# hyunjik11/GPT

Hardware: AMD Instinct MI355X
Metric: SGLD steps/sec (kin40k, n_feat=500/dim, r=5) (higher is better)
Workload: dtype f64

## Files before the change

gpt_amd/csrc/chain.hip:

```cpp
#include "device_util.h"

namespace gpt {

constexpr int kChainBufs = 1;
constexpr int kChainDMax = 8;
constexpr int kChainTPW8 = 1;
constexpr int kChainTasks = 2;
constexpr int kChainG = 2;
constexpr int kChainQPL = 4;
constexpr int kChainQP = 64 * kChainQPL;
constexpr int kChainRun = 64;
constexpr int kChainRunS = 72;
constexpr int kChainQS = 264;

constexpr int kChainMMax = 256;

GPT_HD constexpr int chain_scratch_dbl(int r) {
  const int s0a = 7 * 4 * r * r, s0b = 64 * 8;
  return (s0a > s0b ? s0a : s0b) + 2 * r * r + 3 * r * r + r;
}
GPT_HD constexpr int al16c(int x) { return (x + 15) & ~15; }

template <int R, int G, int WV = kChainDMax>
struct ChainLds {
  static constexpr int DRG = kChainDMax * R * G;
  static constexpr int TS = 2 * (DRG + G);
  static constexpr int NTMAX = kChainQPL * G;
  static constexpr int o_IT = 0;
  static constexpr int o_w = al16c(o_IT + 4 * kChainQP * kChainDMax);
  static constexpr int o_idx = al16c(o_w + 8 * kChainQP);
  static constexpr int o_y = al16c(o_idx + 4 * kChainMMax);
  static constexpr int o_temp = al16c(o_y + 8 * kChainMMax);
  static constexpr int o_fp = al16c(o_temp + 8 * 2 * TS);
  static constexpr int o_gwp = al16c(o_fp + 8 * kChainQPL * G);
  static constexpr int o_misc = al16c(o_gwp + 8 * NTMAX * 64);
  static constexpr int o_touch = al16c(o_misc + 8 * 16);
  static constexpr int o_un = al16c(o_touch + 256);
  static constexpr int L_dbl = G * kChainQS + WV * G * R * kChainRunS;
  static constexpr int x_dbl = chain_scratch_dbl(R);
  static constexpr int o_tab = al16c(o_un + 8 * (L_dbl > x_dbl * WV ? L_dbl : x_dbl * WV));
  static constexpr bool tab = WV == kChainDMax;
  static constexpr int bytes = al16c(o_tab + (tab ? 8 * 64 : 0));
};

#ifndef CHAIN_TIMELINE
#define CHAIN_TIMELINE 2
#endif

#ifndef CHAIN_SSTAMP
#define CHAIN_SSTAMP 0
#endif
#ifndef CHAIN_STAMPS
#define CHAIN_STAMPS CHAIN_SSTAMP
#endif
#define CHAIN_FENCE() do {} while (0)
#ifndef CHAIN_PRIO
#define CHAIN_PRIO 2
#endif
#define CHAIN_SETPRIO(hi_upper)                                                             \
  do {                                                                                      \
    if (CHAIN_PRIO) {                                                                       \
      if ((k >= 4) == (hi_upper)) __builtin_amdgcn_s_setprio(1);                            \
      else __builtin_amdgcn_s_setprio(0);                                                   \
    }                                                                                       \
  } while (0)
#if !CHAIN_STAMPS
#define CSTAMP(slot) CHAIN_FENCE()
#endif
#if CHAIN_TIMELINE
#define TSTAMP_ANY(i)                                                                       \
  do {                                                                                      \
    if (P.tline && tid == 0 && (i) < kTimelineSteps + 2) {                                  \
      long long* ts_ = P.tline + (size_t)blockIdx.x * kTimeline + 2 * (i);                  \
      ts_[0] = (long long)__builtin_amdgcn_s_memrealtime();                                \
      ts_[1] = (long long)__builtin_amdgcn_s_memtime();                                    \
    }                                                                                       \
  } while (0)
#else
#define TSTAMP_ANY(i) do {} while (0)
#endif
#if CHAIN_TIMELINE == 1
#define TSTAMP(i) TSTAMP_ANY(i)
#else
#define TSTAMP(i) do {} while (0)
#endif
#if CHAIN_STAMPS
#define CSTAMP(slot)                                                                        \
  do {                                                                                      \
    if (P.stamps && tid == 0)                                                               \
      P.stamps[(size_t)blockIdx.x * kStamps + (slot)] = (long long)__builtin_amdgcn_s_memtime(); \
  } while (0)
#endif

#if CHAIN_STAMPS
#define LSTAMP(slot)                                                                        \
  do {                                                                                      \
    if (P.stamps && g0 == 20 && lane == 0 && (k == 0 || k == 4))                            \
      P.stamps[(size_t)(gridDim.x + blockIdx.x) * kStamps + (k ? 8 : 0) + (slot)] =         \
          (long long)__builtin_amdgcn_s_memtime();                                         \
  } while (0)
#else
#define LSTAMP(slot) CHAIN_FENCE()
#endif

#define SSTAMP(slot)                                                                        \
  do {                                                                                      \
    if ((slot) == 4) CHAIN_SETPRIO(false);        \
    if ((slot) == 7) CHAIN_SETPRIO(true);        \
    if (CHAIN_SSTAMP && P.stamps && lane == 0 && (k == 0 || k == 4))                                        \
      P.stamps[(size_t)((2 + (slot) / 8) * gridDim.x + blockIdx.x) * kStamps + (k ? 8 : 0) + \
               (slot) % 8] = (long long)__builtin_amdgcn_s_memtime();                       \
  } while (0)

__device__ __forceinline__ void lds_barrier() {
  asm volatile("s_waitcnt lgkmcnt(0)\n\ts_barrier" ::: "memory");
}

template <int R, int J, int G, int WV>
__global__ __launch_bounds__(64 * WV, WV == 4 ? 2 : 1) void chain_kernel(StepParams P,
                                                                const ChainDesc* chains,
                                                                const long long* __restrict__ tbase,
                                                                int t_local, int nsteps) {
  extern __shared__ __attribute__((aligned(16))) unsigned char smem[];
  __shared__ __attribute__((aligned(16))) double pbuf[kChainBufs * WV * G * 64 * J];
  const ChainDesc* Cp = chains + blockIdx.x;
  const int tid = threadIdx.x, lane = tid & 63, k = uni(tid >> 6);
  const int n = P.n, D = P.D, Q = P.Q, m = P.m, NTH = 64 * D;
  using L = ChainLds<R, G, WV>;
  const int NCH = (Q + 63) / 64, NT = NCH * G;
  int* IT_l = (int*)(smem + L::o_IT);
  double* w_l = (double*)(smem + L::o_w);
  int* idx_l = (int*)(smem + L::o_idx);
  double* y_l = (double*)(smem + L::o_y);
  double* temp_l = (double*)(smem + L::o_temp);
  double* fp_l = (double*)(smem + L::o_fp);
  double* gwp_l = (double*)(smem + L::o_gwp);
  double* misc = (double*)(smem + L::o_misc);
  int* flag = (int*)(misc + 8);
  double* wVr = (double*)(smem + L::o_un);
  double* X = (double*)(smem + L::o_un) + k * L::x_dbl;
  double* xi_l = X;
  double* pw0 = pbuf + k * (kChainBufs * G * 64 * J);
  [[maybe_unused]] double* bscr = wVr + G * kChainQS + k * G * R * kChainRunS;

  TSTAMP_ANY(0);
#if CHAIN_TIMELINE
  if (P.tline && tid == 0) {
    long long* ts_ = P.tline + (size_t)blockIdx.x * kTimeline + kTimeline - 2;
    ts_[0] = (long long)__builtin_amdgcn_s_getreg((31 << 11) | 4);
    ts_[1] = (long long)__builtin_amdgcn_s_getreg((31 << 11) | 20);
  }
#endif
  const long long t0 = tbase[0] + t_local;
  if (t0 >= P.total_steps) return;
  if (__hip_atomic_load(Cp->status, __ATOMIC_RELAXED, __HIP_MEMORY_SCOPE_AGENT) != 0) return;
  CSTAMP(0);
  const long long tend = min(P.total_steps, t0 + (long long)nsteps);

  auto batch_of = [&](long long tt, int& bt) -> const int32_t* {
    const int ee = (int)(tt / P.nb), bb = (int)(tt - (long long)ee * P.nb);
    bt = min(m, P.N - bb * m);
    return Cp->order + (size_t)(ee & 1) * P.N + (size_t)bb * m;
  };
  long long t = t0;
  int Bt;
  const int32_t* ord = batch_of(t, Bt);
  const long long koff = (long long)n * k, rstride = (long long)n * D;
  const double* phi_k = uni_ptr(Cp->phi) + koff;
  auto stage_rows = [&](const int (&rows)[G], int ln, double* pw) {
#pragma unroll
    for (int gg = 0; gg < G; ++gg) {
      const char* rb = (const char*)(phi_k + (long long)rows[gg] * rstride);
      __attribute__((address_space(3))) double* dst =
          (__attribute__((address_space(3))) double*)(pw + gg * 64 * J);
      if constexpr (J >= 2) {
#pragma unroll
        for (int s = 0; s < J / 2; ++s) {
          const unsigned o = min(16u * ln + 1024u * s, 8u * n - 16u);
          __builtin_amdgcn_global_load_lds((const __attribute__((address_space(1))) void*)(rb + o),
                                           (__attribute__((address_space(3))) void*)(dst + 128 * s),
                                           16, 0, 0);
        }
      } else {
#pragma unroll
        for (int s = 0; s < 2; ++s) {
          const unsigned o = min(4u * ln + 256u * s, 8u * n - 4u);
          __builtin_amdgcn_global_load_lds((const __attribute__((address_space(1))) void*)(rb + o),
                                           (__attribute__((address_space(3))) void*)(dst + 32 * s),
                                           4, 0, 0);
        }
      }
    }
// ... 149 lines not shown
      const double wV = ok ? wq * V : 0.0;
      if (ok) wVr[gg * kChainQS + q] = wV;
      vsave[x] = ok ? V : 0.0;
      const double fs = wave_sum(wV);
      if (lane == 0) fp_l[gg * kChainQPL + c] = fs;
    }
    LSTAMP(5);
    lds_barrier();
    LSTAMP(6);
    double res[G];
#pragma unroll
    for (int gg = 0; gg < G; ++gg) {
      double f = fp_l[gg * kChainQPL];
#pragma unroll
      for (int c = 1; c < kChainQPL; ++c) f += fp_l[gg * kChainQPL + c];
      res[gg] = (g0 + gg < Bt) ? y_l[g0 + gg] - f : 0.0;
    }
#pragma unroll
    for (int gg = 0; gg < G; ++gg) {
      const double* wr = wVr + gg * kChainQS;
      double a = wr[gq[0] & 0xffff];
#pragma unroll
      for (int i = 1; i < 8; ++i) a += wr[(gq[i >> 1] >> (16 * (i & 1))) & 0xffff];
      a = (group8_sum(a) * tsl[DRG + G + (k * R + rl) * G + gg]) * res[gg];
      double cc[R];
#pragma unroll
      for (int l = 0; l < R; ++l) cc[l] = readlane_d(a, 8 * l);
#pragma unroll
      for (int jj = 0; jj < J; ++jj) {
        const double pv = p[gg][jj];
#pragma unroll
        for (int l = 0; l < R; ++l) acc[jj][l] = fma(pv, cc[l], acc[jj][l]);
      }
    }
#pragma unroll
    for (int x = 0; x < TPW; ++x) {
      const int task = k + D * x;
      if (task >= NT) break;
      const int gg = task / NCH;
      double rr = res[0];
#pragma unroll
      for (int g2 = 1; g2 < G; ++g2) if (gg == g2) rr = res[g2];
      gw[x] = fma(vsave[x], rr, gw[x]);
    }
    LSTAMP(7);
  }
  CSTAMP(2);

  const ChainDesc* Cq = Cp;
  asm volatile("" : "+s"(Cq));
  const ChainDesc C = *Cq;
  const double cN = (double)P.N / (double)Bt;
  const long long post = t - P.burnin_steps;
  const bool store = post >= 0 && ((post + 1) % P.store_every) == 0;
  const long long slot_s = store ? (post + 1) / P.store_every - 1 : 0;

#pragma unroll
  for (int x = 0; x < TPW; ++x) {
    const int task = k + D * x;
    if (task >= NT) break;
    gwp_l[task * 64 + lane] = gw[x];
  }
  SSTAMP(0);
  __syncthreads();
  SSTAMP(1);
  CHAIN_SETPRIO(true);
  {
    const double inv_sw2 = 1.0 / (C.sigma_w * C.sigma_w);
    const double sqe = sqrt(C.epsw);
    double gn2 = 0.0;
#pragma unroll 1
    for (int q = tid; q < Q; q += NTH) {
      const int c = q >> 6, ln = q & 63;
      double g = 0.0;
      for (int gg = 0; gg < G; ++gg) g += gwp_l[(gg * NCH + c) * 64 + ln];
      const double wq = w_l[q];
      const double gradw = cN * g / C.signal_var - wq * inv_sw2;
      double step = C.epsw * gradw / 2;
      step += sqe * normal_at(C.seed, (uint32_t)q, (uint32_t)t, kWNoise, 0);
      const double wn = wq + step;
      w_l[q] = wn;
      if (t + 1 == tend) gptr_w(C.w)[(size_t)((t + 1) & 1) * Q + q] = wn;
      if (store && C.w_store) gptr_w(C.w_store)[(size_t)slot_s * Q + q] = wn;
      gn2 = fma(gradw, gradw, gn2);
    }
    if (C.diag) {
      gn2 = wave_sum(gn2);
      if (lane == 0) misc[k] = gn2;
    }
  }
  SSTAMP(2);
  int Bn = 0;
  const int32_t* ordn = nullptr;
  if (t + 1 < tend) {
    ordn = batch_of(t + 1, Bn);
    for (int i = tid; i < Bn; i += NTH) {
      const int row = gptr(ordn)[i];
      idx_l[i] = row;
      y_l[i] = gptr(Cp->y)[row];
    }
    int rows0[G];
#pragma unroll
    for (int gg = 0; gg < G; ++gg) rows0[gg] = gptr(ordn)[min(gg, Bn - 1)];
    stage_rows(rows0, lane, pw0);
  }
  CSTAMP(3);
  SSTAMP(3);

  const double cU = cN / C.signal_var;
  const double sq = sqrt(C.epsU);
  double gu2 = 0.0;
  {
    constexpr int NQJ = (J + 3) / 4;
    constexpr int NZ = J >= 4 ? 4 : 2;
    const int NQ = unoise_nq(n);
#pragma unroll 1
    for (int l = 0; l < R; ++l) {
#pragma unroll
      for (int q = 0; q < NQJ; ++q) {
        double z[4];
        if constexpr (L::tab)
          normal_quad_tab<NZ>(C.seed, (uint32_t)((l * NQ + q) * 64 + lane), (uint32_t)t, kUNoise,
                              (uint32_t)k, (const double*)(smem + L::o_tab), z);
        else
          normal_quad<NZ>(C.seed, (uint32_t)((l * NQ + q) * 64 + lane), (uint32_t)t, kUNoise,
                          (uint32_t)k, z);
#pragma unroll
        for (int i = 0; i < NZ; ++i)
          if (4 * q + i < J) xi_l[(4 * q + i) * 64 + lane] = z[i];
      }
#pragma unroll
      for (int L = 0; L < R; ++L) {
        if (l == L) {
#pragma unroll
          for (int jj = 0; jj < J; ++jj) {
            const int j = lane + 64 * jj;
            const double Gv = j < n ? acc[jj][L] * cU : 0.0;
            gu2 = fma(Gv, Gv, gu2);
            acc[jj][L] = j < n ? sq * Gv / 2 + xi_l[jj * 64 + lane] : 0.0;
          }
        }
      }
    }
  }
  if (C.diag) {
    gu2 = wave_sum(gu2);
    if (lane == 0) C.diag[(size_t)t * (1 + D) + 1 + k] = sqrt(gu2);
  }
  CSTAMP(4);
  SSTAMP(4);
  {
    constexpr int NN = 2 * R;
    constexpr int S0 = (7 * NN * NN > 64 * 8) ? 7 * NN * NN : 64 * 8;
    double* X0 = X;
    double* Ec = X + S0;
    double* Mg = Ec + NN * R;
    double* Ag = Mg + R * R;
    double* Sg = Ag + R * R;
    double* nr = Sg + R * R;
    wave_sync();
#pragma unroll
    for (int a = 0; a < R; ++a) {
      double v[R];
#pragma unroll
      for (int bb = 0; bb < R; ++bb) {
        double s0 = 0.0;
#pragma unroll
        for (int jj = 0; jj < J; ++jj) s0 = fma(u[jj][a], acc[jj][bb], s0);
        v[bb] = s0;
      }
      wave_sum_to_lds<R>(v, Mg + a * R);
    }
    wave_sync();
    SSTAMP(5);
#pragma unroll
    for (int bb = 0; bb < R; ++bb) {
      double ms[R];
#pragma unroll
      for (int a = 0; a < R; ++a) ms[a] = Mg[a * R + bb] + Mg[bb * R + a];
#pragma unroll
      for (int jj = 0; jj < J; ++jj) {
        double s = 0.0;
#pragma unroll
        for (int a = 0; a < R; ++a) s = fma(u[jj][a], ms[a], s);
        acc[jj][bb] = acc[jj][bb] - s / 2;
      }
    }
      CSTAMP(5);
      SSTAMP(6);
      {
#pragma unroll
        for (int a = 0; a < R; ++a) {
          double v[R];
#pragma unroll
          for (int bb = 0; bb < R; ++bb) {
            double s1 = 0.0;
            if (bb >= a)
#pragma unroll
              for (int jj = 0; jj < J; ++jj) s1 = fma(acc[jj][a], acc[jj][bb], s1);
            v[bb] = s1;
          }
          wave_sum_to_lds<R>(v, Sg + a * R);
        }
        wave_sync();
        for (int o = lane; o < R * R; o += 64) {
          const int i = o / R, b = o - i * R;
          Ag[o] = (Mg[o] - Mg[b * R + i]) / 2;
          if (i > b) Sg[o] = Sg[b * R + i];
        }
      }
      wave_sync();
      const double tt = sq;
      for (int o = lane; o < NN * NN; o += 64) {
        const int i = o / NN, j = o - i * NN;
        double v;
        if (i < R) v = j < R ? Ag[i * R + j] : -Sg[i * R + (j - R)];
        else v = j < R ? (i - R == j ? 1.0 : 0.0) : Ag[(i - R) * R + (j - R)];
        X0[o] = tt * v;
      }
      wave_sync();
      long long* xst = (CHAIN_SSTAMP && P.stamps && k == 0)
                           ? P.stamps + (size_t)(4 * gridDim.x + blockIdx.x) * kStamps : nullptr;
      const bool bad = wave_expm<NN>(X0, xst);
      SSTAMP(7);
      for (int o = lane; o < NN * R; o += 64) {
        const int a = o / R, l = o - a * R;
        Ec[o] = X0[NN * NN + a * NN + l];
      }
      wave_sync();
      double* X1 = X0;
      for (int o = lane; o < R * R; o += 64) X1[o] = -tt * Ag[o];
      wave_sync();
      wave_expm<R>(X1, xst ? xst + (size_t)gridDim.x * kStamps : nullptr);
      if (bad && lane == 0) flag[0] = 1;
      CSTAMP(6);
      SSTAMP(8);
      const double* mx = X1 + R * R;
      double* F = Mg;
      wave_sync();
      for (int o = lane; o < NN * R; o += 64) {
        const int a = o / R, l = o - a * R;
        double s = 0.0;
#pragma unroll
        for (int c2 = 0; c2 < R; ++c2) s = fma(Ec[a * R + c2], mx[c2 * R + l], s);
        F[o] = s;
      }
      wave_sync();
      SSTAMP(9);
      {
        double Fh[R * R];
#pragma unroll
        for (int x = 0; x < R * R; ++x) Fh[x] = F[x];
#pragma unroll
        for (int jj = 0; jj < J; ++jj) {
          double o[R];
#pragma unroll
          for (int l = 0; l < R; ++l) o[l] = 0.0;
#pragma unroll
          for (int a = 0; a < R; ++a)
#pragma unroll
            for (int l = 0; l < R; ++l) o[l] = fma(u[jj][a], Fh[a * R + l], o[l]);
#pragma unroll
          for (int l = 0; l < R; ++l) u[jj][l] = o[l];
        }
      }
      SSTAMP(10);
      double nrm[R];
#pragma unroll
      for (int l = 0; l < R; ++l) nrm[l] = 0.0;
      {
        double Fh[R * R];
#pragma unroll
        for (int x = 0; x < R * R; ++x) Fh[x] = F[R * R + x];
#pragma unroll
        for (int jj = 0; jj < J; ++jj) {
#pragma unroll
          for (int a = 0; a < R; ++a)
#pragma unroll
            for (int l = 0; l < R; ++l) u[jj][l] = fma(acc[jj][a], Fh[a * R + l], u[jj][l]);
#pragma unroll
          for (int l = 0; l < R; ++l) nrm[l] = fma(u[jj][l], u[jj][l], nrm[l]);
        }
      }
      SSTAMP(11);
      wave_sum_to_lds<R>(nrm, nr);
      wave_sync();
      SSTAMP(12);
#pragma unroll
      for (int l = 0; l < R; ++l) {
        const double isc = 1.0 / sqrt(nr[l]);
#pragma unroll
        for (int jj = 0; jj < J; ++jj) u[jj][l] = u[jj][l] * isc;
      }
    }
    SSTAMP(13);
    if (CHAIN_PRIO) __builtin_amdgcn_s_setprio(0);
    if (CHAIN_STAMPS && P.stamps && lane == 0)
    P.stamps[(size_t)blockIdx.x * kStamps + 8 + k] = (long long)__builtin_amdgcn_s_memtime();
  __syncthreads();
    if (C.diag && tid == 0) {
      double s = 0.0;
      for (int w2 = 0; w2 < D; ++w2) s += misc[w2];
      C.diag[(size_t)t * (1 + D)] = sqrt(s);
    }
    if (flag[0]) {
      if (tid == 0) __hip_atomic_store(C.status, 1, __ATOMIC_RELAXED, __HIP_MEMORY_SCOPE_AGENT);
      return;
    }
    double* Uk = (t + 1 == tend) ? C.U + (size_t)n * R * k : nullptr;
    double* Us = (store && C.U_store) ? C.U_store + ((size_t)slot_s * D + k) * n * R : nullptr;
#pragma unroll
    for (int jj = 0; jj < J; ++jj) {
      const int j = lane + 64 * jj;
      if (j < n)
#pragma unroll
        for (int l = 0; l < R; ++l) {
          if (Uk) gptr_w(Uk)[j + (size_t)n * l] = u[jj][l];
          if (Us) gptr_w(Us)[j + (size_t)n * l] = u[jj][l];
        }
    }
    CSTAMP(7);
    SSTAMP(15);
    TSTAMP(2 + (int)(t - t0));
    if (++t >= tend) break;
    ord = ordn;
    Bt = Bn;
  }
#if CHAIN_TIMELINE == 2
  TSTAMP_ANY(2 + (int)(tend - 1 - t0));
#endif
}

static_assert(contains(ChainWVs{}, kChainDMax), "the wide U phase has one wave per dimension");

static int chain_wv(int D) { return D <= 4 ? 4 : kChainDMax; }
static size_t chain_static_lds(int J, int WV) { return 8 * (size_t)kChainBufs * WV * kChainG * 64 * J; }

static int chain_J(int n) { return n <= 64 ? 1 : (n <= 128 ? 2 : (n <= 256 ? 4 : (n <= 512 ? 8 : 0))); }

size_t chain_lds_bytes(int n, int D, int r, int Q, int m) {
  (void)n; (void)Q; (void)m;
  return with_value_or(ChainRanks{}, r, (size_t)1 << 30, [&](auto R) {
    return with_value_or(ChainWVs{}, chain_wv(D), (size_t)1 << 30, [&](auto WV) {
      return (size_t)ChainLds<R, kChainG, WV>::bytes;
    });
  });
}

bool chain_supported(int n, int D, int r, int Q, int m, bool langevin, bool stiefel, int max_run) {
  if (max_run > kChainRun) return false;
  if (!langevin || !stiefel) return false;
  if (D < 1 || D > kChainDMax || r < 1 || r > 5 || chain_J(n) == 0) return false;
  if (chain_J(n) >= 2 && (n & 1)) return false;
  if (Q > kChainQP || m > kChainMMax) return false;
  const int NT = (Q + 63) / 64 * kChainG;
  if (NT > ((chain_J(n) >= 8 && D > 4) ? kChainTPW8 : kChainTasks) * D) return false;
  return chain_lds_bytes(n, D, r, Q, m) + chain_static_lds(chain_J(n), chain_wv(D)) <= 160 * 1024;
}

hipError_t launch_chain(const StepParams& P, const ChainDesc* chains, int nchains,
                        const long long* tbase, int t_local, int nsteps, hipStream_t st) {
  const int J = chain_J(P.n);
  const size_t lds = chain_lds_bytes(P.n, P.D, P.r, P.Q, P.m);
  dim3 grid(nchains), block(64 * P.D);
  return with_value(ChainRanks{}, P.r, [&](auto R) {
    return with_value(ChainJs{}, J, [&](auto JJ) {
      return with_value(ChainWVs{}, chain_wv(P.D), [&](auto WV) {
        return launch_big_lds<chain_kernel<R, JJ, kChainG, WV>>(
            (int)(kMaxLds - chain_static_lds(JJ, WV)), grid, block, lds, st, P, chains, tbase,
            t_local, nsteps);
      });
    });
  });
}

}
```

gpt_amd/csrc/device_util.h:

```cpp
#pragma once
#include "gpt_internal.h"

namespace gpt {

__device__ __forceinline__ int uni(int x) { return __builtin_amdgcn_readfirstlane(x); }
template <class T>
__device__ __forceinline__ T* uni_ptr(T* p) {
  const unsigned long long v = (unsigned long long)p;
  const unsigned lo = __builtin_amdgcn_readfirstlane((unsigned)v);
  const unsigned hi = __builtin_amdgcn_readfirstlane((unsigned)(v >> 32));
  return (T*)(((unsigned long long)hi << 32) | lo);
}

typedef double d4 __attribute__((ext_vector_type(4)));
typedef double d2 __attribute__((ext_vector_type(2)));

__device__ __forceinline__ void tri_pair(long long t, int& a, int& b) {
  int ta = (int)((sqrt(8.0 * (double)t + 1.0) - 1.0) / 2.0);
  while ((long long)ta * (ta + 1) / 2 > t) --ta;
  while ((long long)(ta + 1) * (ta + 2) / 2 <= t) ++ta;
  a = ta;
  b = (int)(t - (long long)ta * (ta + 1) / 2);
}

// ... 516 lines not shown
        for (int x = 0; x < BS; ++x) {
          a[x] = A[min(i0 + x, NN - 1) * NN + t];
          b[x] = B[t * NN + min(j0 + x, NN - 1)];
        }
#pragma unroll
        for (int x = 0; x < BS; ++x)
#pragma unroll
          for (int y = 0; y < BS; ++y) acc[x][y] = fma(a[x], b[y], acc[x][y]);
      }
#pragma unroll
      for (int x = 0; x < BS; ++x)
#pragma unroll
        for (int y = 0; y < BS; ++y)
          if (i0 + x < NN && j0 + y < NN) C[(i0 + x) * NN + j0 + y] = acc[x][y];
    }
    wave_sync();
    return;
  }
  for (int o = lane; o < NN * NN; o += 64) {
    const int i = o / NN, j = o - i * NN;
    double a[NN], b[NN];
#pragma unroll
    for (int t = 0; t < NN; ++t) { a[t] = A[i * NN + t]; b[t] = B[t * NN + j]; }
    double s = 0.0;
#pragma unroll
    for (int t = 0; t < NN; ++t) s = fma(a[t], b[t], s);
    C[o] = s;
  }
  wave_sync();
}

template <int NN>
__device__ __forceinline__ void wave_solve_body(double* M, double* X, long long* st);
template <int NN>
__device__ __noinline__ void wave_solve_ool(double* M, double* X, long long* st) {
  __builtin_assume(__builtin_amdgcn_is_shared((const __attribute__((address_space(0))) void*)M));
  __builtin_assume(__builtin_amdgcn_is_shared((const __attribute__((address_space(0))) void*)X));
  wave_solve_body<NN>(M, X, st);
}
template <int NN>
__device__ __forceinline__ void wave_solve(double* M, double* X, long long* st = nullptr) {
  if constexpr (NN >= 16) wave_solve_ool<NN>(M, X, st);
  else wave_solve_body<NN>(M, X, st);
}
template <int NN>
__device__ __forceinline__ void wave_solve_body(double* M, double* X, long long* st) {
  const int lane = threadIdx.x & 63;
  bool dd = true;
  if (lane < NN) {
    double off = 0.0;
    for (int i = 0; i < NN; ++i)
      if (i != lane) off += fabs(M[i * NN + lane]);
    dd = fabs(M[lane * NN + lane]) > off;
  }
  const bool nopiv = __all(dd);
  for (int c = 0; c < NN; ++c) {
    int bi = c;
    if (!nopiv) {
      const double mine = (lane >= c && lane < NN) ? fabs(M[lane * NN + c]) : -1.0;
      const double best = wave_max(mine);
      const unsigned long long hit = __ballot(mine == best && lane >= c && lane < NN);
      bi = hit ? (int)__ffsll((long long)hit) - 1 : c;
    }
    if (bi != c) {
      for (int col = lane; col < NN; col += 64) {
        double t0 = M[c * NN + col]; M[c * NN + col] = M[bi * NN + col]; M[bi * NN + col] = t0;
        double t1 = X[c * NN + col]; X[c * NN + col] = X[bi * NN + col]; X[bi * NN + col] = t1;
      }
      wave_sync();
    }
    const double rp = 1.0 / M[c * NN + c];
    const int mcols = NN - c - 1, wcols = mcols + NN;
    if (lane < wcols) {
      const int cb = lane + 64;
      const bool two = cb < wcols;
      double* pa = lane < mcols ? M + (c + 1 + lane) : X + (lane - mcols);
      double* pb = two ? (cb < mcols ? M + (c + 1 + cb) : X + (cb - mcols)) : pa;
      const double piva = pa[c * NN], pivb = pb[c * NN];
      for (int r0 = c + 1; r0 < NN; r0 += 8) {
        double fv[8], ca[8], cbv[8];
#pragma unroll
        for (int u = 0; u < 8; ++u) {
          const int rr = min(r0 + u, NN - 1);
          fv[u] = M[rr * NN + c];
          ca[u] = pa[rr * NN];
          cbv[u] = pb[rr * NN];
        }
#pragma unroll
        for (int u = 0; u < 8; ++u) {
          const double f = fv[u] * rp;
          if (r0 + u < NN) {
            pa[(r0 + u) * NN] = ca[u] - f * piva;
            if (two) pb[(r0 + u) * NN] = cbv[u] - f * pivb;
          }
        }
      }
    }
    wave_sync();
  }
  if (st && lane == 0) st[15] = (long long)__builtin_amdgcn_s_memtime();
  for (int col = lane; col < NN; col += 64) {
    double x[NN];
#pragma unroll
    for (int t = 0; t < NN; ++t) x[t] = X[t * NN + col];
#pragma unroll
    for (int c = NN - 1; c >= 0; --c) {
      double s = x[c];
#pragma unroll
      for (int t = c + 1; t < NN; ++t) s -= M[c * NN + t] * x[t];
      x[c] = s / M[c * NN + c];
    }
#pragma unroll
    for (int t = 0; t < NN; ++t) X[t * NN + col] = x[t];
  }
  wave_sync();
}

template <int NV>
__device__ __forceinline__ void wave_sum_to_lds(double (&v)[NV], double* dst) {
  constexpr int NB = NV <= 8 ? 8 : (NV <= 16 ? 16 : (NV <= 32 ? 32 : 64));
  const int lane = lane_id();
  double b[NB];
#pragma unroll
  for (int x = 0; x < NB; ++x) b[x] = x < NV ? v[x] : 0.0;
  Butterfly<NB>::run(b, lane);
  constexpr int SH = 6 - Butterfly<NB>::P;
  const int vi = lane >> SH;
  if ((lane & ((1 << SH) - 1)) == 0 && vi < NV) dst[vi] = b[0];
}
template <int NV>
__device__ __forceinline__ void wave_sum_to_lds(double (&v)[2 * NV], double* dst, double* dst2) {
  constexpr int NB = 2 * NV <= 8 ? 8 : (2 * NV <= 16 ? 16 : (2 * NV <= 32 ? 32 : 64));
  const int lane = lane_id();
  double b[NB];
#pragma unroll
  for (int x = 0; x < NB; ++x) b[x] = x < 2 * NV ? v[x] : 0.0;
  Butterfly<NB>::run(b, lane);
  constexpr int SH = 6 - Butterfly<NB>::P;
  const int vi = lane >> SH;
  if ((lane & ((1 << SH) - 1)) == 0 && vi < 2 * NV) {
    if (vi < NV) dst[vi] = b[0];
    else dst2[vi - NV] = b[0];
  }
}

__device__ __forceinline__ double readlane_d(double v, int lane) {
  const long long b = __double_as_longlong(v);
  const int lo = __builtin_amdgcn_readlane((int)(b & 0xffffffffLL), lane);
  const int hi = __builtin_amdgcn_readlane((int)(b >> 32), lane);
  return __longlong_as_double(((long long)hi << 32) | (unsigned int)lo);
}

template <int NN>
__device__ __forceinline__ bool wave_solve_dd(const double* M, double* X) {
  const int lane = threadIdx.x & 63;
  bool dd = true;
  if (lane < NN) {
    double off = 0.0;
#pragma unroll
    for (int i = 0; i < NN; ++i)
      if (i != lane) off += fabs(M[i * NN + lane]);
    dd = fabs(M[lane * NN + lane]) > off;
  }
  if (!__all(dd)) return false;
  double col[NN];
#pragma unroll
  for (int i = 0; i < NN; ++i) {
    const int c = lane < NN ? lane : lane - NN;
    col[i] = lane < NN ? M[i * NN + c] : (lane < 2 * NN ? X[i * NN + c] : 0.0);
  }
  double rpv[NN];
#pragma unroll
  for (int p = 0; p < NN; ++p) {
    const double rp = rcp_nr(readlane_d(col[p], p));
    rpv[p] = rp;
#pragma unroll
    for (int i = p + 1; i < NN; ++i) {
      const double f = readlane_d(col[i], p) * rp;
      col[i] -= f * col[p];
    }
  }
  const bool xl = lane >= NN;
#pragma unroll
  for (int k = NN - 1; k >= 0; --k) {
    double u[NN];
#pragma unroll
    for (int i = 0; i < k; ++i) u[i] = readlane_d(col[i], k);
    if (xl) {
      col[k] = col[k] * rpv[k];
#pragma unroll
      for (int i = 0; i < k; ++i) col[i] -= col[k] * u[i];
    }
  }
  wave_sync();
  if (lane >= NN && lane < 2 * NN) {
#pragma unroll
    for (int i = 0; i < NN; ++i) X[i * NN + lane - NN] = col[i];
  }
  wave_sync();
  return true;
}

template <int NN>
__device__ __noinline__ bool wave_solve_dd2(const double* Mg, double* Xg, double* Fg) {
  static_assert(NN > 32 && NN <= 64, "two-pass register LU");
  typedef __attribute__((address_space(3))) double lds_d;
  const lds_d* M = (const lds_d*)Mg;
  lds_d* X = (lds_d*)Xg;
  lds_d* F = (lds_d*)Fg;
  const int lane = lane_id();
  bool dd = true;
  if (lane < NN) {
    double off = 0.0;
#pragma unroll
    for (int i = 0; i < NN; ++i)
      if (i != lane) off += fabs(M[i * NN + lane]);
    dd = fabs(M[lane * NN + lane]) > off;
  }
  if (!__all(dd)) return false;
  double col[NN];
#pragma unroll
  for (int i = 0; i < NN; ++i) col[i] = M[i * NN + (lane < NN ? lane : 0)];
#pragma unroll
  for (int p = 0; p < NN; ++p) {
    if (lane == p) {
      const double rp = rcp_nr(col[p]);
      F[p * NN + p] = rp;
#pragma unroll
      for (int i = p + 1; i < NN; ++i) F[i * NN + p] = col[i] * rp;
    }
    wave_sync();
#pragma unroll
    for (int i = p + 1; i < NN; ++i) col[i] -= F[i * NN + p] * col[p];
  }
#pragma unroll
  for (int i = 0; i < NN - 1; ++i)
    if (i < lane && lane < NN) F[i * NN + lane] = col[i];
  wave_sync();
#pragma unroll
  for (int i = 0; i < NN; ++i) col[i] = X[i * NN + (lane < NN ? lane : 0)];
#pragma unroll
  for (int p = 0; p < NN; ++p) {
    int zo = 0;
    asm volatile("" : "+v"(zo) : "v"(col[p]));
#pragma unroll
    for (int i = p + 1; i < NN; ++i) col[i] -= F[zo + i * NN + p] * col[p];
  }
#pragma unroll
  for (int k = NN - 1; k >= 0; --k) {
    int zo = 0;
    asm volatile("" : "+v"(zo) : "v"(col[k]));
    col[k] = col[k] * F[zo + k * NN + k];
#pragma unroll
    for (int i = 0; i < k; ++i) col[i] -= col[k] * F[zo + i * NN + k];
  }
  wave_sync();
  if (lane < NN) {
#pragma unroll
    for (int i = 0; i < NN; ++i) X[i * NN + lane] = col[i];
  }
  wave_sync();
  return true;
}

template <int NN, bool kRegLU2 = true>
__device__ bool wave_expm(double* S, long long* st = nullptr) {
  __builtin_assume(__builtin_amdgcn_is_shared((const __attribute__((address_space(0))) void*)S));
  const int lane = threadIdx.x & 63;
#define GPT_XST(i)                                                        \
  do {                                                                    \
    if (st && lane == 0) st[i] = (long long)__builtin_amdgcn_s_memtime(); \
  } while (0)
  GPT_XST(11);
  constexpr int q = NN * NN;
  double* A = S;
  double* A2 = S + q;
  double* A4 = S + 2 * q;
  double* A6 = S + 3 * q;
  double* U = S + 4 * q;
  double* V = S + 5 * q;
  double* T = S + 6 * q;
  double cs = 0.0;
  if (lane < NN) {
#pragma unroll
    for (int i = 0; i < NN; ++i) cs += fabs(A[i * NN + lane]);
  }
  if (__any(!(cs <= 1.79769313486231570e308))) {
    for (int o = lane; o < q; o += 64) A2[o] = __builtin_nan("");
    wave_sync();
    return true;
  }
  const double nA = wave_max(cs);
  int si = 0;
  if (nA <= 2.1) {
    const int deg = nA > 0.95 ? 9 : (nA > 0.25 ? 7 : (nA > 0.015 ? 5 : 3));
    if (st && lane == 0) st[10] = deg;
    const double* C = kPade[(deg - 3) / 2];
    wave_mm<NN>(A, A, A2);
    const double c0 = C[0], c1 = C[1];
    for (int o = lane; o < q; o += 64) {
      const double id = (o / NN == o - (o / NN) * NN) ? 1.0 : 0.0;
      T[o] = id;
      U[o] = c1 * id;
      V[o] = c0 * id;
    }
    wave_sync();
    for (int kk = 1; kk <= (deg - 1) / 2; ++kk) {
      if (kk > 1) wave_mm<NN>(T, A2, A4);
      const double* Pk = kk > 1 ? A4 : A2;
      const double cu = C[2 * kk + 1], cv = C[2 * kk];
      for (int o = lane; o < q; o += 64) {
        const double p = Pk[o];
        T[o] = p;
        U[o] = U[o] + cu * p;
        V[o] = V[o] + cv * p;
      }
      wave_sync();
    }
    wave_mm<NN>(A, U, A6);
    for (int o = lane; o < q; o += 64) U[o] = A6[o];
    wave_sync();
  } else {
    const double s = log2(nA / 5.4);
    si = (s > 0.0) ? (int)ceil(s) : 0;
    if (st && lane == 0) st[10] = 13 + 100 * si;
    if (si > 0) {
      const double sc = ldexp(1.0, -si);
      for (int o = lane; o < q; o += 64) A[o] *= sc;
      wave_sync();
    }
    constexpr double c[14] = {64764752532480000.0, 32382376266240000.0, 7771770303897600.0,
                              1187353796428800.0, 129060195264000.0, 10559470521600.0,
                              670442572800.0, 33522128640.0, 1323241920.0, 40840800.0, 960960.0,
                              16380.0, 182.0, 1.0};
    wave_mm<NN>(A, A, A2);
    wave_mm<NN>(A2, A2, A4);
    wave_mm<NN>(A2, A4, A6);
    for (int o = lane; o < q; o += 64) T[o] = c[13] * A6[o] + c[11] * A4[o] + c[9] * A2[o];
    wave_sync();
    wave_mm<NN>(A6, T, V);
    for (int o = lane; o < q; o += 64) {
      const double id = (o / NN == o - (o / NN) * NN) ? 1.0 : 0.0;
      V[o] = V[o] + c[7] * A6[o] + c[5] * A4[o] + c[3] * A2[o] + c[1] * id;
      T[o] = c[12] * A6[o] + c[10] * A4[o] + c[8] * A2[o];
    }
    wave_sync();
    wave_mm<NN>(A, V, U);
    wave_mm<NN>(A6, T, V);
    for (int o = lane; o < q; o += 64) {
      const double id = (o / NN == o - (o / NN) * NN) ? 1.0 : 0.0;
      V[o] = V[o] + c[6] * A6[o] + c[4] * A4[o] + c[2] * A2[o] + c[0] * id;
    }
    wave_sync();
  }
  GPT_XST(12);
  double* M = A4;
  double* X = A2;
  for (int o = lane; o < q; o += 64) {
    M[o] = V[o] - U[o];
    X[o] = V[o] + U[o];
  }
  wave_sync();
  bool solved = false;
  if constexpr (2 * NN <= 64) solved = wave_solve_dd<NN>(M, X);
  else if constexpr (kRegLU2 && NN <= 64) solved = wave_solve_dd2<NN>(M, X, U);
  if (!solved) wave_solve<NN>(M, X, st);
  GPT_XST(13);
  for (int z = 0; z < si; ++z) {
    wave_mm<NN>(X, X, T);
    for (int o = lane; o < q; o += 64) X[o] = T[o];
    wave_sync();
  }
  GPT_XST(14);
#undef GPT_XST
  bool bad = false;
  for (int o = lane; o < q; o += 64) bad |= (X[o] != X[o]);
  return __any(bad);
}

}
```

gpt_amd/csrc/wave.hip:

```cpp
#include "device_util.h"

namespace gpt {

template <int NN>
struct Blk {
  static constexpr int BS = (NN + 7) / 8, NB = (NN + BS - 1) / BS;
  double v[BS][BS];
};

template <int NN>
__device__ __forceinline__ void blk_origin(int lane, int& i0, int& j0) {
  constexpr int BS = Blk<NN>::BS, NB = Blk<NN>::NB;
  i0 = min(lane / NB, NB - 1) * BS;
  j0 = (lane % NB) * BS;
}

template <int NN>
__device__ __forceinline__ void blk_mm(const double* A, const double* B, Blk<NN>& C, int lane) {
  constexpr int BS = Blk<NN>::BS;
  int i0, j0;
  blk_origin<NN>(lane, i0, j0);
#pragma unroll
  for (int x = 0; x < BS; ++x)
#pragma unroll
// ... 867 lines not shown
    double x[4][J];
#pragma unroll
    for (int da = 0; da < 4; ++da)
#pragma unroll
      for (int jj = 0; jj < J; ++jj) {
        const int a = a0 + da;
        const double* src = a < R ? Ug + (size_t)n * a : park + (size_t)n * (a - R);
        x[da][jj] = a < 2 * R ? gptr(src)[jc[jj]] : 0.0;
      }
#pragma unroll
    for (int da = 0; da < 4; ++da) {
      const int a = a0 + da;
      if (a < 2 * R) {
        double f[R];
#pragma unroll
        for (int l = 0; l < R; ++l) f[l] = F[a * R + l];
#pragma unroll
        for (int jj = 0; jj < J; ++jj) {
          const double xa = jok[jj] ? x[da][jj] : 0.0;
#pragma unroll
          for (int l = 0; l < R; ++l) u[jj][l] = fma(xa, f[l], u[jj][l]);
        }
      }
    }
    __builtin_amdgcn_sched_barrier(0);
  }
  double nrm[R];
#pragma unroll
  for (int l = 0; l < R; ++l) {
    nrm[l] = 0.0;
#pragma unroll
    for (int jj = 0; jj < J; ++jj) nrm[l] = fma(u[jj][l], u[jj][l], nrm[l]);
  }
  double* nr = S2 + R * R;
  wv_sum_to_lds<R>(nrm, nr, lane);
  wave_sync();
#pragma unroll
  for (int l = 0; l < R; ++l) {
    const double isc = 1.0 / sqrt(nr[l]);
#pragma unroll
    for (int jj = 0; jj < J; ++jj) u[jj][l] = u[jj][l] * isc;
  }
  {
    const long long post = t - P.burnin_steps;
    const bool store = post >= 0 && ((post + 1) % P.store_every) == 0;
    const long long slot = store ? (post + 1) / P.store_every - 1 : 0;
    double* Us = (store && Cp->U_store) ? Cp->U_store + ((size_t)slot * D + k) * n * R : nullptr;
#pragma unroll
    for (int jj = 0; jj < J; ++jj)
      if (jok[jj]) {
#pragma unroll
        for (int l = 0; l < R; ++l) {
          gptr_w(Ug)[jc[jj] + (size_t)n * l] = u[jj][l];
          if (Us) gptr_w(Us)[jc[jj] + (size_t)n * l] = u[jj][l];
        }
      }
  }
  WSTAMP(srow, 10);
  const long long t1 = t + 1;
  if (t1 < P.total_steps) {
    const int e1 = (int)(t1 / P.nb), b1 = (int)(t1 - (long long)e1 * P.nb);
    const int B1 = min(m, P.N - b1 * m);
    const int32_t* ord1 = Cp->order + (size_t)(e1 & 1) * P.N + (size_t)b1 * m;
    double* tdst = Cp->temp + (size_t)(t1 & 1) * D * R * m;
    if ((n & 1) == 0) {
      wave_sync();
      u_to_lds();
      phidotU_mfma(ord1, B1, tdst);
    } else {
      phidotU(ord1, B1, tdst);
    }
  }
  WSTAMP(srow, 11);
}

static int wv_J(int n) { return n <= 64 ? 1 : (n <= 128 ? 2 : (n <= 192 ? 3 : (n <= 256 ? 4 : 0))); }

size_t wv_dim_lds_bytes(int n, int r, int m) { return 8 * ((size_t)wv_dim_lds_dbl(n, r, m) + 64); }
size_t wv_vphase_lds_bytes(int D, int r, int Q, int m) {
  return 8 * (size_t)wv_vphase_lds_dbl(D, r, Q, m);
}

bool wave_supported(int n, int D, int r, int Q, int m, bool langevin, bool stiefel) {
  if (!langevin || !stiefel) return false;
  if (!contains(WaveRanks{}, r) || wv_J(n) == 0 || m > kWvMaxM || D < 1 || D > kDMax) return false;
  if (3 * r * r > n * r) return false;
  if ((long long)D * r * m >= 65536 || Q >= 65536) return false;
  return wv_vphase_lds_bytes(D, r, Q, m) <= 160 * 1024 && wv_dim_lds_bytes(n, r, m) <= 160 * 1024;
}

void wave_tables(const std::vector<int32_t>& I0, int Q, int D, int r, int m,
                 std::vector<uint16_t>& out) {
  out.assign((size_t)wv_table_shorts(D, r, Q), 0);
  for (int q = 0; q < Q; ++q)
    for (int k = 0; k < D; ++k)
      out[(size_t)q * D + k] = (uint16_t)((k * r + I0[q + (size_t)Q * k]) * m);
  uint16_t* mem = out.data() + (size_t)Q * D;
  for (int k = 0; k < D; ++k) {
    int pos = 0;
    uint16_t* seg = mem + (size_t)D * Q + (size_t)k * (r + 1);
    for (int l = 0; l < r; ++l) {
      seg[l] = (uint16_t)pos;
      for (int q = 0; q < Q; ++q)
        if (I0[q + (size_t)Q * k] == l) mem[(size_t)k * Q + pos++] = (uint16_t)q;
    }
    seg[r] = (uint16_t)pos;
  }
}

hipError_t launch_wave(const StepParams& P, const ChainDesc* chains, int nchains,
                       const long long* tbase, int t_local, bool init, hipStream_t st) {
  const int J = wv_J(P.n);
  const size_t ldsv = wv_vphase_lds_bytes(P.D, P.r, P.Q, P.m);
  const size_t ldsd = wv_dim_lds_bytes(P.n, P.r, P.m);
  return with_value(WaveRanks{}, P.r, [&](auto R) {
    if (!init) {
      const hipError_t e = launch_big_lds<wv_vphase_kernel<R>>(
          kMaxLds, dim3(nchains), dim3(512), ldsv, st, P, chains, tbase, t_local);
      if (e != hipSuccess) return e;
    }
    return with_value(WaveJs{}, J, [&](auto JJ) {
      return launch_big_lds<wv_dim_kernel<R, JJ>>(kMaxLds, dim3(nchains * P.D), dim3(64), ldsd, st,
                                                  P, chains, tbase, t_local, nchains,
                                                  init ? 1 : 0);
    });
  });
}

}

namespace gpt {
template <int NN, int MODE>
__global__ __launch_bounds__(64) void wv_expm_check_kernel(const double* A, double* E, int32_t* bad,
                                                           long long* st) {
  extern __shared__ __attribute__((aligned(16))) double wv_sm[];
  const int lane = lane_id();
  const double* a = A + (size_t)blockIdx.x * NN * NN;
  double* S0 = wv_sm;
  for (int o = lane; o < NN * NN; o += 64) S0[o] = a[o];
  wave_sync();
  bool b;
  const double* res = S0 + NN * NN;
  if constexpr (MODE == 2) {
    long long* sm = st ? st + 4 * (size_t)blockIdx.x : nullptr;
    if (sm && lane == 0) sm[0] = (long long)__builtin_amdgcn_s_memtime();
    b = wv_expm<NN>(S0, S0 + NN * NN, S0 + 2 * NN * NN, lane, sm ? sm + 1 : nullptr, NN / 2);
    if (sm && lane == 0) sm[3] = (long long)__builtin_amdgcn_s_memtime();
  } else if constexpr (MODE == 0) {
    b = wv_expm<NN>(S0, S0 + NN * NN, S0 + 2 * NN * NN, lane);
  } else if constexpr (MODE == 4) {
    b = wv_expm<NN>(S0, S0 + NN * NN, S0 + 2 * NN * NN, lane, nullptr, NN / 2);
  } else if constexpr (MODE == 3) {
    b = wave_expm<NN, false>(S0);
  } else {
    b = wave_expm<NN>(S0);
  }
  wave_sync();
  for (int o = lane; o < NN * NN; o += 64) E[(size_t)blockIdx.x * NN * NN + o] = res[o];
  if (lane == 0) bad[blockIdx.x] = b ? 1 : 0;
}

template <int NN, int MODE>
static hipError_t expm_check_launch(int count, const double* A, double* E, int32_t* bad,
                                    hipStream_t st, long long* stamps) {
  const size_t lds = 8 * (size_t)(MODE == 1 || MODE == 3 ? 7 : 3) * NN * NN;
  hipError_t e = hipFuncSetAttribute((const void*)wv_expm_check_kernel<NN, MODE>,
                                     hipFuncAttributeMaxDynamicSharedMemorySize, 160 * 1024);
  if (e != hipSuccess) return e;
  hipLaunchKernelGGL((wv_expm_check_kernel<NN, MODE>), dim3(count), dim3(64), lds, st, A, E, bad,
                     stamps);
  return hipGetLastError();
}

hipError_t launch_expm_check(int nn, int count, const double* A, double* E, int32_t* bad, int mode,
                             hipStream_t st, long long* stamps) {
  const auto go = [&](auto MODE, auto sizes) {
    return with_value(sizes, nn, [&](auto NN) {
      return expm_check_launch<NN, MODE>(count, A, E, bad, st, stamps);
    });
  };
  using Geod = IntList<12, 16, 20, 24, 30, 32, 40>;
  switch (mode) {
    case 0: return go(Int<0>{}, IntList<6, 8, 10, 12, 15, 16, 20, 24, 30, 32, 40>{});
    case 1: return go(Int<1>{}, IntList<1, 2, 3, 4, 5, 6, 8, 10, 12, 15, 16, 20, 24, 30, 32, 40>{});
    case 2: return go(Int<2>{}, Geod{});
    case 3: return go(Int<3>{}, IntList<40>{});
    case 4: return go(Int<4>{}, Geod{});
    default: return hipErrorInvalidValue;
  }
}
}
```

Before: 3.065 million.

## Evaluate small-matrix Pade polynomial in registers and trim chain expm staging

For small matrices (NN<=10, which includes the 2R=10 and R=5 expm calls in the SGLD chain step), the Pade polynomial is now accumulated in per-lane registers using a register-tiled matmul. This replaces the LDS-based loop with its repeated stores and wave syncs, and the NaN check is folded into the diagonally-dominant solve. The chain step now builds the antisymmetric part inline while assembling X0, writes the X1 exponent input into a dedicated scratch region, and reads the Ec block straight from the expm output. That removes several copy passes and syncs, at the cost of a larger LDS scratch footprint per wave. A test mode is added that keeps the old polynomial path for comparison.

```diff
diff --git a/gpt_amd/csrc/chain.hip b/gpt_amd/csrc/chain.hip
--- a/gpt_amd/csrc/chain.hip
+++ b/gpt_amd/csrc/chain.hip
@@ -15,9 +15,9 @@
 
 constexpr int kChainMMax = 256;
 
-GPT_HD constexpr int chain_scratch_dbl(int r) {
+GPT_HD constexpr int chain_scratch_dbl(int r, bool own_x1) {
   const int s0a = 7 * 4 * r * r, s0b = 64 * 8;
-  return (s0a > s0b ? s0a : s0b) + 2 * r * r + 3 * r * r + r;
+  return (s0a > s0b ? s0a : s0b) + (own_x1 ? 7 : 2) * r * r + 3 * r * r + r;
 }
 GPT_HD constexpr int al16c(int x) { return (x + 15) & ~15; }
 
@@ -37,7 +37,8 @@
   static constexpr int o_touch = al16c(o_misc + 8 * 16);
   static constexpr int o_un = al16c(o_touch + 256);
   static constexpr int L_dbl = G * kChainQS + WV * G * R * kChainRunS;
-  static constexpr int x_dbl = chain_scratch_dbl(R);
+  static constexpr bool own_x1 = WV == kChainDMax;
+  static constexpr int x_dbl = chain_scratch_dbl(R, own_x1);
   static constexpr int o_tab = al16c(o_un + 8 * (L_dbl > x_dbl * WV ? L_dbl : x_dbl * WV));
   static constexpr bool tab = WV == kChainDMax;
   static constexpr int bytes = al16c(o_tab + (tab ? 8 * 64 : 0));
@@ -493,9 +494,11 @@
   {
     constexpr int NN = 2 * R;
     constexpr int S0 = (7 * NN * NN > 64 * 8) ? 7 * NN * NN : 64 * 8;
+    constexpr bool kOwnX1 = L::own_x1;
     double* X0 = X;
     double* Ec = X + S0;
-    double* Mg = Ec + NN * R;
+    double* X1 = kOwnX1 ? X + S0 : X0;
+    double* Mg = X + S0 + (kOwnX1 ? 7 * R * R : NN * R);
     double* Ag = Mg + R * R;
     double* Sg = Ag + R * R;
     double* nr = Sg + R * R;
@@ -543,47 +546,48 @@
           }
           wave_sum_to_lds<R>(v, Sg + a * R);
         }
-        wave_sync();
-        for (int o = lane; o < R * R; o += 64) {
-          const int i = o / R, b = o - i * R;
-          Ag[o] = (Mg[o] - Mg[b * R + i]) / 2;
-          if (i > b) Sg[o] = Sg[b * R + i];
-        }
       }
       wave_sync();
       const double tt = sq;
       for (int o = lane; o < NN * NN; o += 64) {
         const int i = o / NN, j = o - i * NN;
+        const int ia = i < R ? i : i - R, ja = j < R ? j : j - R;
+        const double a = (Mg[ia * R + ja] - Mg[ja * R + ia]) / 2;
         double v;
-        if (i < R) v = j < R ? Ag[i * R + j] : -Sg[i * R + (j - R)];
-        else v = j < R ? (i - R == j ? 1.0 : 0.0) : Ag[(i - R) * R + (j - R)];
+        if (i < R) v = j < R ? a : -Sg[ia <= ja ? ia * R + ja : ja * R + ia];
+        else v = j < R ? (ia == j ? 1.0 : 0.0) : a;
         X0[o] = tt * v;
+        if (kOwnX1 && i < R && j < R) X1[ia * R + ja] = -tt * a;
+        if (!kOwnX1 && i < R && j < R) Ag[ia * R + ja] = a;
       }
       wave_sync();
       long long* xst = (CHAIN_SSTAMP && P.stamps && k == 0)
                            ? P.stamps + (size_t)(4 * gridDim.x + blockIdx.x) * kStamps : nullptr;
       const bool bad = wave_expm<NN>(X0, xst);
       SSTAMP(7);
-      for (int o = lane; o < NN * R; o += 64) {
-        const int a = o / R, l = o - a * R;
-        Ec[o] = X0[NN * NN + a * NN + l];
-      }
-      wave_sync();
-      double* X1 = X0;
-      for (int o = lane; o < R * R; o += 64) X1[o] = -tt * Ag[o];
-      wave_sync();
+      if constexpr (!kOwnX1) {
+        for (int o = lane; o < NN * R; o += 64) {
+          const int a = o / R, l = o - a * R;
+          Ec[o] = X0[NN * NN + a * NN + l];
+        }
+        wave_sync();
+        for (int o = lane; o < R * R; o += 64) X1[o] = -tt * Ag[o];
+        wave_sync();
+      }
       wave_expm<R>(X1, xst ? xst + (size_t)gridDim.x * kStamps : nullptr);
       if (bad && lane == 0) flag[0] = 1;
       CSTAMP(6);
       SSTAMP(8);
       const double* mx = X1 + R * R;
       double* F = Mg;
+      const double* El = kOwnX1 ? X0 + NN * NN : Ec;
+      constexpr int ES = kOwnX1 ? NN : R;
       wave_sync();
       for (int o = lane; o < NN * R; o += 64) {
         const int a = o / R, l = o - a * R;
         double s = 0.0;
 #pragma unroll
-        for (int c2 = 0; c2 < R; ++c2) s = fma(Ec[a * R + c2], mx[c2 * R + l], s);
+        for (int c2 = 0; c2 < R; ++c2) s = fma(El[a * ES + c2], mx[c2 * R + l], s);
         F[o] = s;
       }
       wave_sync();
diff --git a/gpt_amd/csrc/device_util.h b/gpt_amd/csrc/device_util.h
--- a/gpt_amd/csrc/device_util.h
+++ b/gpt_amd/csrc/device_util.h
@@ -692,7 +692,7 @@
 }
 
 template <int NN>
-__device__ __forceinline__ bool wave_solve_dd(const double* M, double* X) {
+__device__ __forceinline__ bool wave_solve_dd(const double* M, double* X, bool* nan = nullptr) {
   const int lane = threadIdx.x & 63;
   bool dd = true;
   if (lane < NN) {
@@ -736,6 +736,12 @@
   if (lane >= NN && lane < 2 * NN) {
 #pragma unroll
     for (int i = 0; i < NN; ++i) X[i * NN + lane - NN] = col[i];
+  }
+  if (nan) {
+    bool b = false;
+#pragma unroll
+    for (int i = 0; i < NN; ++i) b |= (col[i] != col[i]);
+    *nan = __any(b && lane >= NN && lane < 2 * NN);
   }
   wave_sync();
   return true;
@@ -803,8 +809,88 @@
   return true;
 }
 
-template <int NN, bool kRegLU2 = true>
+template <int NN>
+struct PadeReg {
+  static constexpr int BC = NN > 8 ? 2 : 1, NL = NN * NN / BC;
+  static constexpr bool ok = NN <= 10 && NN % BC == 0 && NL <= 64;
+};
+
+template <int NN, int BC, int NH>
+__device__ __forceinline__ void wave_mm_reg(const double* A, const double* B, int i, int j0,
+                                            double (&c)[BC]) {
+  constexpr int TH = (NN + NH - 1) / NH;
+#pragma unroll
+  for (int y = 0; y < BC; ++y) c[y] = 0.0;
+#pragma unroll
+  for (int h = 0; h < NH; ++h) {
+    if (h) __builtin_amdgcn_sched_barrier(0);
+    double a[TH], b[TH][BC];
+#pragma unroll
+    for (int t = 0; t < TH; ++t)
+      if (h * TH + t < NN) a[t] = A[i * NN + h * TH + t];
+#pragma unroll
+    for (int t = 0; t < TH; ++t)
+#pragma unroll
+      for (int y = 0; y < BC; ++y)
+        if (h * TH + t < NN) b[t][y] = B[(h * TH + t) * NN + j0 + y];
+#pragma unroll
+    for (int y = 0; y < BC; ++y)
+#pragma unroll
+      for (int t = 0; t < TH; ++t)
+        if (h * TH + t < NN) c[y] = fma(a[t], b[t][y], c[y]);
+  }
+}
+
+template <int NN>
+__device__ __forceinline__ void wave_pade_reg(double* S, const double* C, int K) {
+  constexpr int BC = PadeReg<NN>::BC, NL = PadeReg<NN>::NL, q = NN * NN;
+  const int lane = threadIdx.x & 63;
+  const int o0 = lane < NL ? lane * BC : 0;
+  const int i = o0 / NN, j0 = o0 - i * NN;
+  double* A2 = S + q;
+  constexpr int NH = NN > 8 ? 2 : 1, NHL = NN > 8 ? 3 : 1;
+  double P[BC], U[BC], V[BC];
+  wave_mm_reg<NN, BC, NH>(S, S, i, j0, P);
+  {
+    const double c0 = C[0], c1 = C[1], cv = C[2], cu = C[3];
+#pragma unroll
+    for (int y = 0; y < BC; ++y) {
+      const bool d = i == j0 + y;
+      const double u0 = d ? c1 : 0.0, v0 = d ? c0 : 0.0;
+      U[y] = u0 + cu * P[y];
+      V[y] = v0 + cv * P[y];
+    }
+  }
+  double* Pk = A2;
+  for (int kk = 2; kk <= K; ++kk) {
+#pragma unroll
+    for (int y = 0; y < BC; ++y) Pk[o0 + y] = P[y];
+    wave_sync();
+    wave_mm_reg<NN, BC, NHL>(Pk, A2, i, j0, P);
+    const double cu = C[2 * kk + 1], cv = C[2 * kk];
+#pragma unroll
+    for (int y = 0; y < BC; ++y) {
+      U[y] = U[y] + cu * P[y];
+      V[y] = V[y] + cv * P[y];
+    }
+    Pk = kk == 2 ? S + 2 * q : S + 6 * q;
+  }
+  double* Ub = S + 4 * q;
+#pragma unroll
+  for (int y = 0; y < BC; ++y) Ub[o0 + y] = U[y];
+  wave_sync();
+  wave_mm_reg<NN, BC, NH>(S, Ub, i, j0, U);
+#pragma unroll
+  for (int y = 0; y < BC; ++y) {
+    S[2 * q + o0 + y] = V[y] - U[y];
+    S[q + o0 + y] = V[y] + U[y];
+  }
+  wave_sync();
+}
+
+template <int NN, bool kRegLU2 = true, bool kRegPoly = true>
 __device__ bool wave_expm(double* S, long long* st = nullptr) {
+  constexpr bool kReg = kRegPoly && PadeReg<NN>::ok;
   __builtin_assume(__builtin_amdgcn_is_shared((const __attribute__((address_space(0))) void*)S));
   const int lane = threadIdx.x & 63;
 #define GPT_XST(i)                                                        \
@@ -832,34 +918,40 @@
   }
   const double nA = wave_max(cs);
   int si = 0;
+  bool mx = false;
   if (nA <= 2.1) {
     const int deg = nA > 0.95 ? 9 : (nA > 0.25 ? 7 : (nA > 0.015 ? 5 : 3));
     if (st && lane == 0) st[10] = deg;
     const double* C = kPade[(deg - 3) / 2];
-    wave_mm<NN>(A, A, A2);
-    const double c0 = C[0], c1 = C[1];
-    for (int o = lane; o < q; o += 64) {
-      const double id = (o / NN == o - (o / NN) * NN) ? 1.0 : 0.0;
-      T[o] = id;
-      U[o] = c1 * id;
-      V[o] = c0 * id;
-    }
-    wave_sync();
-    for (int kk = 1; kk <= (deg - 1) / 2; ++kk) {
-      if (kk > 1) wave_mm<NN>(T, A2, A4);
-      const double* Pk = kk > 1 ? A4 : A2;
-      const double cu = C[2 * kk + 1], cv = C[2 * kk];
+    if constexpr (kReg) {
+      wave_pade_reg<NN>(S, C, (deg - 1) / 2);
+      mx = true;
+    } else {
+      wave_mm<NN>(A, A, A2);
+      const double c0 = C[0], c1 = C[1];
       for (int o = lane; o < q; o += 64) {
-        const double p = Pk[o];
-        T[o] = p;
-        U[o] = U[o] + cu * p;
-        V[o] = V[o] + cv * p;
+        const double id = (o / NN == o - (o / NN) * NN) ? 1.0 : 0.0;
+        T[o] = id;
+        U[o] = c1 * id;
+        V[o] = c0 * id;
       }
       wave_sync();
-    }
-    wave_mm<NN>(A, U, A6);
-    for (int o = lane; o < q; o += 64) U[o] = A6[o];
-    wave_sync();
+      for (int kk = 1; kk <= (deg - 1) / 2; ++kk) {
+        if (kk > 1) wave_mm<NN>(T, A2, A4);
+        const double* Pk = kk > 1 ? A4 : A2;
+        const double cu = C[2 * kk + 1], cv = C[2 * kk];
+        for (int o = lane; o < q; o += 64) {
+          const double p = Pk[o];
+          T[o] = p;
+          U[o] = U[o] + cu * p;
+          V[o] = V[o] + cv * p;
+        }
+        wave_sync();
+      }
+      wave_mm<NN>(A, U, A6);
+      for (int o = lane; o < q; o += 64) U[o] = A6[o];
+      wave_sync();
+    }
   } else {
     const double s = log2(nA / 5.4);
     si = (s > 0.0) ? (int)ceil(s) : 0;
@@ -896,13 +988,15 @@
   GPT_XST(12);
   double* M = A4;
   double* X = A2;
-  for (int o = lane; o < q; o += 64) {
-    M[o] = V[o] - U[o];
-    X[o] = V[o] + U[o];
-  }
-  wave_sync();
-  bool solved = false;
-  if constexpr (2 * NN <= 64) solved = wave_solve_dd<NN>(M, X);
+  if (!mx) {
+    for (int o = lane; o < q; o += 64) {
+      M[o] = V[o] - U[o];
+      X[o] = V[o] + U[o];
+    }
+    wave_sync();
+  }
+  bool solved = false, nanx = false;
+  if constexpr (2 * NN <= 64) solved = wave_solve_dd<NN>(M, X, kReg ? &nanx : nullptr);
   else if constexpr (kRegLU2 && NN <= 64) solved = wave_solve_dd2<NN>(M, X, U);
   if (!solved) wave_solve<NN>(M, X, st);
   GPT_XST(13);
@@ -913,6 +1007,7 @@
   }
   GPT_XST(14);
 #undef GPT_XST
+  if (kReg && solved && si == 0) return nanx;
   bool bad = false;
   for (int o = lane; o < q; o += 64) bad |= (X[o] != X[o]);
   return __any(bad);
diff --git a/gpt_amd/csrc/wave.hip b/gpt_amd/csrc/wave.hip
--- a/gpt_amd/csrc/wave.hip
+++ b/gpt_amd/csrc/wave.hip
@@ -1043,6 +1043,8 @@
     b = wv_expm<NN>(S0, S0 + NN * NN, S0 + 2 * NN * NN, lane, nullptr, NN / 2);
   } else if constexpr (MODE == 3) {
     b = wave_expm<NN, false>(S0);
+  } else if constexpr (MODE == 5) {
+    b = wave_expm<NN, true, false>(S0);
   } else {
     b = wave_expm<NN>(S0);
   }
@@ -1054,7 +1056,7 @@
 template <int NN, int MODE>
 static hipError_t expm_check_launch(int count, const double* A, double* E, int32_t* bad,
                                     hipStream_t st, long long* stamps) {
-  const size_t lds = 8 * (size_t)(MODE == 1 || MODE == 3 ? 7 : 3) * NN * NN;
+  const size_t lds = 8 * (size_t)(MODE == 1 || MODE == 3 || MODE == 5 ? 7 : 3) * NN * NN;
   hipError_t e = hipFuncSetAttribute((const void*)wv_expm_check_kernel<NN, MODE>,
                                      hipFuncAttributeMaxDynamicSharedMemorySize, 160 * 1024);
   if (e != hipSuccess) return e;
@@ -1077,6 +1079,7 @@
     case 2: return go(Int<2>{}, Geod{});
     case 3: return go(Int<3>{}, IntList<40>{});
     case 4: return go(Int<4>{}, Geod{});
+    case 5: return go(Int<5>{}, IntList<1, 2, 3, 4, 5, 6, 8, 10>{});
     default: return hipErrorInvalidValue;
   }
 }
```

Result: faster. 3.097 million (median of 6 runs) (+1.1%).
